# pbluc/avrecode-ms

Measured on AMD Instinct MI355X. Metric: H.264 bytes/s recompressed (CABAC re-encode of recorded bin streams, bit-exact vs CPU), higher is better.
Workload: dtype u32

## Files before the change

### avrecode-ms_amd/csrc/avr_k1p.h

```cpp
#pragma once
#include <stdint.h>

#include "avr_chunk.h"

#if defined(__HIPCC__)
#define AVR_HD __host__ __device__ inline
#else
#define AVR_HD inline
#endif

namespace avr {
namespace k1p {

#if defined(__HIP_DEVICE_COMPILE__)
#define AVR_PIN2(a, b) asm volatile("" : "+v"(a), "+v"(b))
#else
#define AVR_PIN2(a, b) ((void)0)
#endif

constexpr uint32_t kNone = 0xffffffffu;
constexpr uint32_t kMaxStretch = 16 * kChunk;
constexpr uint32_t kCodeBypass = 252;
constexpr uint32_t kCodePad = 252;

// ... 217 lines not shown
    if (chunk == 0) {
        o->first = 0;
        R[0] = R[1] = R[2] = R[3] = 510;
        i = 0;
    } else {
        uint32_t f = kNone;
        const uint32_t hi = limit < n ? limit : n;
        for_codes(res, lo, hi, [&](uint32_t idx, uint32_t c) { if (code_is_boundary(c)) { f = idx; return true; } return false; });
        if (f == kNone) {
            o->first = kNone; o->end = 0;
            for (int q = 0; q < 4; q++) { o->t_exit[q] = 0; o->r_exit[q] = 0; }
            return;
        }
        o->first = f;
        const uint32_t row = codes[res[f]].row;
        for (uint32_t q = 0; q < 4; q++) { uint32_t sh; R[q] = post_lps_range(row, q, &sh); }
        i = f + 1;
    }
    bool closed = false;
    auto merged = [&]() { return R[0] == R[1] && R[1] == R[2] && R[2] == R[3]; };
    auto code_by_code = [&](uint32_t stop) {
        if (i >= stop) return;
        uint32_t i_next = stop;
        for_codes(res, i, stop, [&](uint32_t idx, uint32_t c) {
            if (merged()) { i_next = idx; return true; }
            const bool closing = idx >= limit && code_is_boundary(c);
            if (closing)
                for (uint32_t q = 0; q < 4; q++) o->exit_q |= uint8_t(((R[q] >> 6) & 3) << (2 * q));
            const CodeEntry e = codes[c];
            for (uint32_t q = 0; q < 4; q++) T[q] += step_range(e, &R[q]);
            i_next = idx + 1;
            if (closing) { closed = true; return true; }
            return false;
        });
        i = i_next;
    };
    {
        const uint32_t interior_end = limit < n ? limit : n;
        const uint32_t a16 = (i + 15) & ~15u;
        code_by_code(a16 < interior_end ? a16 : interior_end);
        while (!merged() && i + 16 <= interior_end) {
            const U4 v = *reinterpret_cast<const U4 *>(res + i);
            const uint32_t w[4] = {v.x, v.y, v.z, v.w};
#if defined(__HIP_DEVICE_COMPILE__)
#pragma unroll 1
#endif
            for (uint32_t k = 0; k < 4; k++) {
                CodeEntry e[4];
                code_entries4(codes, w[k], e);
                for (uint32_t b = 0; b < 4; b++)
                    for (uint32_t q = 0; q < 4; q++) T[q] += step_range(e[b], &R[q]);
            }
            i += 16;
        }
        code_by_code(n);
    }
    uint32_t Rm = R[0], Tm = 0, end = i;
    if (!closed && i < n) {
        const uint32_t interior_end = limit < n ? limit : n;
        if (i < interior_end) {
            for_codes_all(res, i, interior_end, [&](uint32_t c) { Tm += step_range(codes[c], &Rm); },
                          [&](uint32_t d) {
                              CodeEntry e[4];
                              code_entries4(codes, d, e);
                              Tm += step_range(e[0], &Rm); Tm += step_range(e[1], &Rm);
                              Tm += step_range(e[2], &Rm); Tm += step_range(e[3], &Rm);
                          });
            i = interior_end;
        }
        end = n;
        for_codes(res, i, n, [&](uint32_t idx, uint32_t c) {
            const bool closing = idx >= limit && code_is_boundary(c);
            if (closing) o->exit_q = uint8_t(((Rm >> 6) & 3) * 0x55u);
            Tm += step_range(codes[c], &Rm);
            if (closing) { end = idx + 1; return true; }
            if (idx - lo > max_stretch) { o->too_long = 1; end = idx + 1; return true; }
            return false;
        });
        R[0] = R[1] = R[2] = R[3] = Rm;
    }
    o->end = end;
    for (uint32_t q = 0; q < 4; q++) { o->t_exit[q] = T[q] + Tm; o->r_exit[q] = uint16_t(R[q]); }
}


struct Entry {
    uint32_t t_start;
    uint32_t q;
};

struct SliceTotals {
    uint32_t t_total;
    uint32_t r_final;
    uint32_t bad;
    uint32_t pad;
};

AVR_HD void b2_chain(const Stretch *st, uint32_t n_chunks, Entry *en, SliceTotals *tot) {
    uint32_t T = 0, q = 0, r = 510, bad = 0;
    for (uint32_t c = 0; c < n_chunks; c++) {
        if (st[c].first == kNone) continue;
        en[c].t_start = T;
        en[c].q = q;
        T += st[c].t_exit[q];
        r = st[c].r_exit[q];
        bad |= st[c].too_long;
        q = (st[c].exit_q >> (2 * q)) & 3;
    }
    tot->t_total = T;
    tot->r_final = r;
    tot->bad = bad;
    tot->pad = 0;
}

AVR_HD uint32_t ref_digits(uint32_t t) { return t <= 21 ? 0 : (t - 21 + 15) / 16; }


template <class A, class = void> struct adder_is_staged { static constexpr bool value = false; };
template <class A> struct adder_is_staged<A, decltype(void(A::kStaged))> { static constexpr bool value = A::kStaged; };
template <class Src, class Adder>
AVR_HD void c_stretch_in(const Src &src, const Stretch &st, const Entry &en, uint32_t chunk,
                         const CodeEntryC *codes, Adder &S) {
    uint32_t R, from;
    if (chunk == 0) { R = 510; from = 0; }
    else { uint32_t sh; R = post_lps_range(codes[src.byte(st.first)].row, en.q, &sh); from = st.first + 1; }
    const uint32_t phase = en.t_start & 15, g0 = en.t_start >> 4;
    uint64_t L2 = 0;
    int sp = int(phase) - 7;
    uint32_t j = 0;
    constexpr bool staged = adder_is_staged<Adder>::value;
    if constexpr (staged) S.begin(g0);
    auto bin_e = [&](const CodeEntryC &e) {
        uint32_t v;
        const uint32_t sh = step_range_c(e, &R, &v);
        L2 = (L2 + v) << sh;
        sp += int(sh);
    };
    auto bin = [&](uint32_t c) { bin_e(codes[c]); };
    auto put = [&](uint32_t d) {
        if constexpr (staged) S.push(g0 + j, d);
        else if (j < 2) S.add(g0 + j, d);
        else S.store(g0 + j, d);
        j++;
    };
    auto digits = [&]() {
        while (sp >= 15) {
            const uint32_t d = uint32_t(L2 >> (sp + 1));
            L2 &= (uint64_t(2) << sp) - 1;
            put(d);
            sp -= 16;
        }
    };
    auto digits2 = [&]() {
        const int s1 = sp + 1;
        const uint32_t nd = uint32_t(s1 > 0 ? s1 : 0) >> 4, ks = 16 + (uint32_t(s1) & 15u);
        const uint64_t t = L2 >> ks;
        const uint32_t a = nd == 2 ? uint32_t(t >> 16) : uint32_t(t), b = uint32_t(t) & 0xffffu;
        L2 = uint32_t(L2) & (nd ? (1u << ks) - 1 : ~0u);
        sp -= int(16 * nd);
        if constexpr (staged) { S.push2(nd, a, b); j += nd; S.look(g0 + j); }
        else { if (nd) put(a); if (nd == 2) put(b); }
    };
    const uint32_t to = st.end;
    if (from < to) {
        auto four = [&](uint32_t d) {
            CodeEntryC e[4];
// ... 76 lines not shown
```

### avrecode-ms_amd/csrc/avr_k1p.hip

```cpp
#include <hip/hip_runtime.h>

#include <mutex>
#include <stdint.h>
#include <stdlib.h>
#include <type_traits>

#include "avr_coder.h"
#include "avr_internal.h"
#include "avr_k1p.h"
#include "avr_tables.h"

namespace avr {

static __device__ const CabacTables d_tables = make_cabac_tables();

using namespace k1p;

struct Plan {
    const uint16_t *recs;
    const uint64_t *rec_off;
    const uint32_t *n_bins;
    const uint64_t *res_off;
    const uint32_t *chunk_base, *chunk_slice;
    const uint32_t *blk_base, *blk_slice;
// ... 384 lines not shown
    uint64_t bits0 = 0, bits1 = 0;
    ChainAhead ahead(lbits, lend, nk, k, c0);
    ahead.walk(n_ch, [&](const ChainAhead::Chunk &c) {
        if (st[0] == st[1]) {
            *eo = uint8_t(st[0]);
            met_chunk = met_chunk < at ? met_chunk : at;
            if (at < 0xffffu) n_bins = kSegBits + 1u;
        }
        eo += row4;
        at++;
        const uint32_t cnt = c.cnt;
        const bool room = n_bins < kSegBits && cnt;
        if (__any(room) && room) {
            const uint32_t sh = c.pos & 31u;
            const uint64_t lo = uint64_t(__builtin_amdgcn_alignbit(c.w.y, c.w.x, sh)) | uint64_t(__builtin_amdgcn_alignbit(c.w.z, c.w.y, sh)) << 32;
            const uint64_t got = cnt < 64u ? lo & ((uint64_t(1) << cnt) - 1) : lo;
            if (n_bins < 64u) { bits0 |= got << n_bins; bits1 |= n_bins ? got >> (64u - n_bins) : 0u; }
            else bits1 |= got << (n_bins - 64u);
        }
        n_bins += cnt > 64u ? kSegBits + 1u : cnt;
        chain_step<2>(tn, c.bw, c.pos, cnt, c.w, st);
    });
    SegSummary o;
    o.bits[0] = bits0; o.bits[1] = bits1; o.n_bins = n_bins; o.exit_state = uint8_t(st[0]); o.met = st[0] == st[1] && met_chunk < 0xffffu;
    o.met_chunk = uint16_t(met_chunk < 0xffffu ? met_chunk : 0xffffu);
    summ[(size_t(L.s) * nk + k) * n_segs + L.seg] = o;
}

template <bool NOTE>
__device__ __forceinline__ uint32_t chain_chunks(const uint8_t *tn, const uint32_t *lbits, const uint16_t *lend, uint8_t *est, uint32_t nk, uint32_t row4,
                                                 uint32_t k, uint32_t c_first, uint32_t n_ch, uint32_t st0) {
    uint8_t *eo = est + size_t(c_first) * row4 + k;
    uint32_t st[1] = {st0};
    ChainAhead ahead(lbits, lend, nk, k, c_first);
    ahead.walk(n_ch, [&](const ChainAhead::Chunk &c) {
        if (NOTE) { *eo = uint8_t(st[0]); eo += row4; }
        chain_step<1>(tn, c.bw, c.pos, st[0] < 126u ? c.cnt : 0u, c.w, st);
    });
    return st[0];
}

__global__ __launch_bounds__(64 * kSegWaves) void k_k1p_chain_fix(Plan p, uint32_t n_slices, uint32_t n_segs, const int32_t *status,
                                                       const uint8_t *tng, const uint32_t *lbits, const uint16_t *lend, const uint8_t *init_states,
                                                       uint8_t *est, const SegSummary *summ, uint8_t *final_states, uint32_t force_walk_every) {
    __shared__ uint8_t tn[kTnBytes];
    for (uint32_t i = threadIdx.x; i < kTnBytes / 16; i += 64 * kSegWaves) reinterpret_cast<uint4 *>(tn)[i] = reinterpret_cast<const uint4 *>(tng)[i];
    __syncthreads();
    ChainLane L;
    if (!chain_lane(p, n_slices, n_segs, status, &L)) return;
    const uint32_t nk = p.n_states, row4 = ((nk + 3) >> 2) << 2, k = L.k;
    const SegSummary *mine = summ + (size_t(L.s) * nk + k) * n_segs;
    const uint32_t init = init_states[size_t(L.s) * p.ns_full + L.col] & 127u;
    const uint32_t c_slice = p.chunk_base[L.s], seg_len = (L.nc + n_segs - 1) / n_segs;
    const bool distrust = force_walk_every && (L.s * nk + k) % force_walk_every == 0;
    uint32_t from = L.seg, entry = init;
    if (init < 126u) {
        while (from > 0 && (distrust || !mine[from - 1].met)) from--;
        if (from > 0) entry = mine[from - 1].exit_state;
        for (uint32_t g = from; g < L.seg; g++) {
            const SegSummary sg = mine[g];
            if (sg.n_bins <= kSegBits && !distrust) {
                uint64_t b = sg.bits[0], b_hi = sg.bits[1];
                for (uint32_t left = sg.n_bins; left;) {
                    const uint32_t n = left < 8u ? left : 8u;
                    entry = tn[(128u << n) - 128u + (entry << n) + (uint32_t(b) & ((1u << n) - 1u))];
                    b = (b >> 8) | (b_hi << 56); b_hi >>= 8; left -= n;
                }
            } else {
                const uint32_t g_begin = g * seg_len < L.nc ? g * seg_len : L.nc, g_end = g_begin + seg_len < L.nc ? g_begin + seg_len : L.nc;
                entry = chain_chunks<false>(tn, lbits, lend, est, nk, row4, k, c_slice + g_begin, g_end - g_begin, entry);
            }
        }
    }
    const SegSummary me = mine[L.seg];
    const uint32_t n_ch = L.c_end - L.c_begin;
    const bool met = me.met && init < 126u && !distrust;
    const uint32_t stop = met && me.met_chunk < n_ch ? me.met_chunk : n_ch;
    const uint32_t exit_state = chain_chunks<true>(tn, lbits, lend, est, nk, row4, k, c_slice + L.c_begin, stop, entry);
    if (final_states && (L.c_end == L.nc) && (L.c_begin < L.nc || L.seg == 0))
        final_states[size_t(L.s) * p.ns_full + L.col] = uint8_t(stop < n_ch ? me.exit_state : exit_state);
}

__device__ __forceinline__ CodeEntry device_code_entry(uint32_t c);
__device__ __forceinline__ uint2 device_codes2(uint32_t c);

constexpr uint32_t kStBypass = 128, kStTerminate = 129, kStPad = 130, kStNone = 131, kReplayStates = 132;

typedef uint16_t u16x2 __attribute__((ext_vector_type(2)));
__device__ __forceinline__ uint32_t pk_sub(uint32_t a, uint32_t b) { return __builtin_bit_cast(uint32_t, __builtin_bit_cast(u16x2, a) - __builtin_bit_cast(u16x2, b)); }
__device__ __forceinline__ uint32_t pk_add(uint32_t a, uint32_t b) { return __builtin_bit_cast(uint32_t, __builtin_bit_cast(u16x2, a) + __builtin_bit_cast(u16x2, b)); }
__device__ __forceinline__ uint32_t pk_shl(uint32_t a, uint32_t b) { return __builtin_bit_cast(uint32_t, __builtin_bit_cast(u16x2, a) << __builtin_bit_cast(u16x2, b)); }
__device__ __forceinline__ uint32_t pk_shr8(uint32_t a) { return (a >> 8) & 0x00ff00ffu; }
__device__ __forceinline__ uint32_t step_pair(uint32_t &Rp, uint32_t row, uint32_t rown, uint32_t shrow, bool sym, uint32_t extra) {
    const uint32_t sel = ((Rp >> 6) & 0x00030003u) | 0x0c000c00u;
    const uint32_t rl = __builtin_amdgcn_perm(row, row, sel);
    const uint32_t rm = pk_sub(Rp, rl);
    const uint32_t shm = pk_shr8(rm) ^ 0x00010001u;
    const uint32_t rn = __builtin_amdgcn_perm(rown, rown, sel) | 0x01000100u;
    const uint32_t shl = __builtin_amdgcn_perm(shrow, shrow, sel);
    Rp = sym ? rn : pk_shl(rm, shm);
    return (sym ? shl : shm) + extra;
}

struct B1Walk {
    uint32_t i0, i1, limit, n, max_stretch;
    const uint2 *codes2;
    uint32_t mode, Rp0, Rp1, Tp0, Tp1, T[4], Rm, Tm, end;
    bool merged;
    Stretch o;

    __device__ __forceinline__ void init(uint32_t chunk, uint32_t i0_, uint32_t i1_, uint32_t n_, uint32_t max_stretch_, const uint2 *codes2_) {
        i0 = i0_; i1 = i1_; limit = i0_ + kChunk; n = n_; max_stretch = max_stretch_; codes2 = codes2_;
        mode = 0; Rp0 = Rp1 = 0x01fe01feu; Tp0 = Tp1 = 0; T[0] = T[1] = T[2] = T[3] = 0; Rm = 510; Tm = 0; end = 0;
        merged = false;
        o.first = kNone; o.end = 0; o.exit_q = 0; o.too_long = 0; o.pad[0] = o.pad[1] = 0;
        for (int q = 0; q < 4; q++) { o.t_exit[q] = 0; o.r_exit[q] = 0; }
        if (chunk == 0) { o.first = 0; mode = 2; merged = true; }
    }
    __device__ __forceinline__ void flush_t() {
        T[0] += Tp0 & 0xffffu; T[1] += Tp0 >> 16; T[2] += Tp1 & 0xffffu; T[3] += Tp1 >> 16;
        Tp0 = Tp1 = 0;
    }
    __device__ __forceinline__ bool met() const { return Rp0 == Rp1 && (Rp0 >> 16) == (Rp0 & 0xffffu); }
    __device__ __forceinline__ void one(uint32_t idx, const uint4 &e) {
        const CodeEntry ce{e.x, e.y >> 16};
        const bool boundary = ce.meta & 1u;
        if (mode == 0) {
            if (idx < i1 && boundary) {
                o.first = idx;
                const uint32_t rown = codes2[(e.y >> 8) & 0xffu].x;
                Rp0 = __builtin_amdgcn_perm(rown, rown, 0x0c010c00u) | 0x01000100u;
                Rp1 = __builtin_amdgcn_perm(rown, rown, 0x0c030c02u) | 0x01000100u;
                mode = 1;
            }
        } else if (mode == 1) {
            const bool closing = idx >= limit && boundary;
            if (closing)
                o.exit_q |= uint8_t(((Rp0 >> 6) & 3u) | ((Rp0 >> 22) & 3u) << 2 | ((Rp1 >> 6) & 3u) << 4 | ((Rp1 >> 22) & 3u) << 6);
            const uint2 e2 = codes2[(e.y >> 8) & 0xffu];
            const uint32_t extra = (ce.meta >> 8) * 0x00010001u;
            Tp0 = pk_add(Tp0, step_pair(Rp0, ce.row, e2.x, e2.y, boundary, extra));
            Tp1 = pk_add(Tp1, step_pair(Rp1, ce.row, e2.x, e2.y, boundary, extra));
            if (closing) { end = idx + 1; mode = 3; }
            else if (met()) { Rm = Rp0 & 0xffffu; mode = 2; merged = true; }
        } else if (mode == 2) {
            const bool closing = idx >= limit && boundary;
            if (closing) o.exit_q = uint8_t(((Rm >> 6) & 3) * 0x55u);
            Tm += step_merged(e);
            if (closing) { end = idx + 1; mode = 3; }
            else if (idx >= limit && idx - i0 > max_stretch) { o.too_long = 1; end = idx + 1; mode = 3; }
        }
    }
    __device__ __forceinline__ uint32_t step_merged(const uint4 &e) {
        uint32_t v;
        return step_range_c(CodeEntryC{e.x, e.z, 0u, e.w}, &Rm, &v);
    }
    __device__ __forceinline__ void group(uint32_t base, const uint4 e[8]) {
        if (mode == 2 && base + 8 <= i1) {
#pragma unroll
            for (uint32_t j = 0; j < 8; j++) Tm += step_merged(e[j]);
        } else if (mode == 1 && base + 8 <= i1) {
#pragma unroll
            for (uint32_t j = 0; j < 8; j++) {
                const uint2 e2 = codes2[(e[j].y >> 8) & 0xffu];
                const bool sym = (e[j].y >> 16) & 1u;
                const uint32_t extra = (e[j].y >> 24) * 0x00010001u;
                Tp0 = pk_add(Tp0, step_pair(Rp0, e[j].x, e2.x, e2.y, sym, extra));
                Tp1 = pk_add(Tp1, step_pair(Rp1, e[j].x, e2.x, e2.y, sym, extra));
            }
            flush_t();
            if (met()) { Rm = Rp0 & 0xffffu; mode = 2; merged = true; }
        } else if (mode != 3) {
            for (uint32_t j = 0; j < 8; j++) if (base + j < n) one(base + j, e[j]);
            flush_t();
        }
    }
    __device__ __forceinline__ void chunk_done() { if (mode == 0) mode = 3; }
    __device__ __forceinline__ void tail(uint32_t base, const uint4 e[8]) {
        for (uint32_t j = 0; j < 8; j++) if (base + j < n && mode != 3) one(base + j, e[j]);
        flush_t();
    }
    __device__ __forceinline__ const Stretch &finish() {
        if (o.first != kNone) {
            o.end = mode != 3 ? n : end;
            for (uint32_t q = 0; q < 4; q++) {
                const uint32_t rq = ((q & 2u) ? Rp1 : Rp0) >> (16 * (q & 1u)) & 0xffffu;
                o.t_exit[q] = T[q] + (merged ? Tm : 0u);
                o.r_exit[q] = uint16_t(merged ? Rm : rq);
            }
        }
        return o;
    }
};

template <bool TILE_CODES, bool R8>
__global__ __launch_bounds__(256) void k_k1p_replay(Plan p, uint32_t total_chunks, const uint32_t *est, uint8_t *res,
                                                    const int32_t *status, Stretch *stretch, uint32_t max_stretch) {
    extern __shared__ uint32_t replay_lds[];
    __shared__ uint4 info[2 * kReplayStates];
    __shared__ uint2 codes2[256];
    constexpr uint32_t kSelOff = R8 ? 128 : 2048;
    __shared__ uint32_t sel_off[kSelOff];
    const uint32_t lane = threadIdx.x & 63, nk = p.n_states;
    for (uint32_t c = threadIdx.x; c < 256; c += blockDim.x) codes2[c] = device_codes2(c);
    uint8_t *stb = reinterpret_cast<uint8_t *>(replay_lds) + (threadIdx.x >> 6) * (((nk + 8) >> 2) << 8) + lane * 4;
    for (uint32_t sel = threadIdx.x; sel < kSelOff; sel += blockDim.x) {
        uint32_t kk;
        if (R8) {
            kk = sel < nk ? sel : sel == AVR_SEL8_BYPASS ? nk + 1 : sel == AVR_SEL8_TERMINATE ? nk + 2 : nk + 4;
        } else {
            const uint32_t kLast = AVR_MAX_STATES - 1, over = (sel < kLast ? kLast : sel > kLast + 4 ? kLast + 4 : sel) - kLast;
            const uint32_t dense = sel < AVR_MAX_STATES ? uint32_t(p.table[sel]) : kNotUsed;
            kk = (dense < nk ? dense : nk) + over;
        }
        sel_off[sel] = ((kk & ~3u) << 6) + (kk & 3u);
    }
    for (uint32_t i = threadIdx.x; i < 2 * kReplayStates; i += blockDim.x) {
        const uint32_t st = i >> 1, bin = i & 1u;
        uint32_t next, code;
        if (st < 128) {
            const uint32_t nx = d_tables.packed[st][1];
            next = ((bin ^ st) & 1u) ? (nx >> 8) & 0xffu : nx & 0xffu;
            code = code_context(st, bin);
        } else {
            next = st;
            code = st == kStBypass ? kCodeBypass | bin : st == kStTerminate ? code_terminate(bin) : kCodePad;
        }
        const CodeEntry ce = device_code_entry(code);
        const CodeEntryC cc = code_entry_c(ce);
        info[i] = make_uint4(ce.row, next | code << 8 | ce.meta << 16, cc.side, cc.adj);
    }
    __syncthreads();
    const uint32_t gc = blockIdx.x * blockDim.x + threadIdx.x;
    if (gc >= total_chunks) return;
    const uint32_t s = p.chunk_slice[gc];
    Stretch o;
    o.first = kNone; o.end = 0; o.exit_q = 0; o.too_long = 0; o.pad[0] = o.pad[1] = 0;
    for (int q = 0; q < 4; q++) { o.t_exit[q] = 0; o.r_exit[q] = 0; }
    if (status[s] != AVR_SLICE_OK) { stretch[gc] = o; return; }
    const uint32_t c = gc - p.chunk_base[s];
    const uint32_t n = p.n_bins[s];
    const ChunkSpan span = chunk_span(c, n);
    const uint32_t i0 = span.i0, i1 = span.i1;
    {
        const uint32_t nkw = (nk + 3) >> 2;
        const uint32_t *e = est + size_t(gc) * nkw;
        for (uint32_t kw = 0; kw < nkw; kw++) *reinterpret_cast<uint32_t *>(stb + kw * 256) = e[kw];
        const uint32_t pseudo[5] = {kStNone, kStBypass, kStTerminate, kStPad, kStNone};
#pragma unroll
        for (uint32_t j = 0; j < 5; j++) stb[((nk + j) >> 2) * 256 + ((nk + j) & 3)] = uint8_t(pseudo[j]);
    }
    const uint16_t *r = p.recs + p.rec_off[s];
    uint8_t *ro = TILE_CODES ? res + TileCodes::group_at(gc, 0) : res + p.res_off[s];
    auto put16 = [&](uint32_t i, const U4 &v) {
        if (TILE_CODES) *reinterpret_cast<U4 *>(ro + size_t((i - i0) >> 4) * kTileRowBytes) = v;
        else *reinterpret_cast<U4 *>(ro + i) = v;
    };
    B1Walk b1;
    b1.init(c, i0, i1, n, max_stretch, codes2);
    auto eight = [&](const U4 &v, uint32_t &c0, uint32_t &c1, uint4 e[8]) {
        const uint32_t w[4] = {v.x, v.y, v.z, v.w};
        uint32_t off[8];
#pragma unroll
        for (uint32_t j = 0; j < 8; j++) off[j] = sel_off[((w[j >> 1] >> ((j & 1) * 16)) >> 1) & 0x7ffu];
#pragma unroll
        for (uint32_t j = 0; j < 8; j++) {
            const uint32_t bin = (w[j >> 1] >> ((j & 1) * 16)) & 1u;
            uint8_t *sp = stb + off[j];
            const uint32_t st = *sp;
            e[j] = info[(st << 1) | bin];
            *sp = uint8_t(e[j].y);
        }
        c0 = __builtin_amdgcn_perm(e[1].y, e[0].y, 0x0c0c0501u) | __builtin_amdgcn_perm(e[3].y, e[2].y, 0x05010c0cu);
        c1 = __builtin_amdgcn_perm(e[5].y, e[4].y, 0x0c0c0501u) | __builtin_amdgcn_perm(e[7].y, e[6].y, 0x05010c0cu);
    };
    if (R8) {
        const uint32_t pad_off = (((nk + 3) & ~3u) << 6) + ((nk + 3) & 3u);
        auto eight8 = [&](uint32_t lo, uint32_t hi, uint32_t base, uint32_t lim, auto masked, uint32_t &c0, uint32_t &c1, uint4 e[8]) {
            uint32_t off[8], bin[8];
#pragma unroll
            for (uint32_t j = 0; j < 8; j++) {
                const uint32_t b = ((j < 4 ? lo : hi) >> (8 * (j & 3))) & 0xffu;
                off[j] = sel_off[b >> 1];
                if (decltype(masked)::value) off[j] = base + j < lim ? off[j] : pad_off;
                bin[j] = b & 1u;
            }
#pragma unroll
            for (uint32_t j = 0; j < 8; j++) {
                uint8_t *sp = stb + off[j];
                const uint32_t st = *sp;
                e[j] = info[(st << 1) | bin[j]];
                *sp = uint8_t(e[j].y);
            }
            c0 = __builtin_amdgcn_perm(e[1].y, e[0].y, 0x0c0c0501u) | __builtin_amdgcn_perm(e[3].y, e[2].y, 0x05010c0cu);
            c1 = __builtin_amdgcn_perm(e[5].y, e[4].y, 0x0c0c0501u) | __builtin_amdgcn_perm(e[7].y, e[6].y, 0x05010c0cu);
        };
        auto sixteen8 = [&](uint32_t base, const U4 &v, auto masked) {
            U4 a;
            uint4 e[8];
            eight8(v.x, v.y, base, i1, masked, a.x, a.y, e); b1.group(base, e);
            eight8(v.z, v.w, base + 8, i1, masked, a.z, a.w, e); b1.group(base + 8, e);
            put16(base, a);
        };
        const uint8_t *r8 = p.recs8 + (p.rec_off[s] & ~uint64_t(15));
        if (i0 < n) {
            for_record_groups8(r8, i0, i1, sixteen8);
            b1.chunk_done();
            for (uint32_t i = i0 + kChunk; b1.mode != 3 && i < n; i += 8) {
                const uint2 v = *reinterpret_cast<const uint2 *>(r8 + i);
                uint32_t c0, c1;
                uint4 e[8];
                eight8(v.x, v.y, i, n, std::true_type{}, c0, c1, e);
                b1.tail(i, e);
            }
        }
        stretch[gc] = b1.finish();
        return;
    }
    uint32_t i = i0;
    if (i0 < n) {
        U4 v0{0, 0, 0, 0}, v1 = v0, v2 = v0, v3 = v0;
        const uint32_t last = i + 32 <= i1 ? i0 + ((i1 - i0) / 32u - 1u) * 32u : i0;
        if (i + 32 <= i1) {
            const U4 *q = reinterpret_cast<const U4 *>(r + i);
            v0 = q[0]; v1 = q[1]; v2 = q[2]; v3 = q[3];
        }
        for (; i + 32 <= i1; i += 32) {
            const U4 *qn = reinterpret_cast<const U4 *>(r + (i + 32 <= last ? i + 32 : last));
            const U4 n0 = qn[0], n1 = qn[1], n2 = qn[2], n3 = qn[3];
            U4 a, b;
            uint4 e[8];
            eight(v0, a.x, a.y, e); b1.group(i, e);
            eight(v1, a.z, a.w, e); b1.group(i + 8, e);
            eight(v2, b.x, b.y, e); b1.group(i + 16, e);
            eight(v3, b.z, b.w, e); b1.group(i + 24, e);
            put16(i, a);
            put16(i + 16, b);
            v0 = n0; v1 = n1; v2 = n2; v3 = n3;
        }
        for (; i < i1; i += 16) {
            const U4 *q = reinterpret_cast<const U4 *>(r + i);
            const U4 nop{AVR_NOP_CABAC2, AVR_NOP_CABAC2, AVR_NOP_CABAC2, AVR_NOP_CABAC2};
            const U4 t0 = q[0], t1 = i + 8 < i1 ? q[1] : nop;
            U4 a;
            uint4 e[8];
            eight(t0, a.x, a.y, e); b1.group(i, e);
            eight(t1, a.z, a.w, e); b1.group(i + 8, e);
            put16(i, a);
        }
        b1.chunk_done();
        for (i = i0 + kChunk; b1.mode != 3 && i < n; i += 8) {
            uint32_t c0, c1;
            uint4 e[8];
            eight(*reinterpret_cast<const U4 *>(r + i), c0, c1, e);
            b1.tail(i, e);
        }
    }
    stretch[gc] = b1.finish();
}


__device__ __forceinline__ CodeEntry device_code_entry(uint32_t c) {
    if (code_is_bypass(c)) return CodeEntry{0u, 0x100u | ((c & 1u) << 1)};
    return CodeEntry{d_tables.packed[2 * (c >> 2)][0], code_sym(c) * 3u};
}

__device__ __forceinline__ uint2 device_codes2(uint32_t c) {
    const uint32_t row = device_code_entry(c).row;
    uint32_t rown = 0, shrow = 0;
    for (uint32_t q = 0; q < 4; q++) {
        const uint32_t rl = (row >> (8 * q)) & 0xffu;
        if (rl) { uint32_t sh; const uint32_t rn = post_lps_range(row, q, &sh); rown |= (rn & 0xffu) << (8 * q); shrow |= sh << (8 * q); }
    }
    return make_uint2(rown, shrow);
}

__global__ __launch_bounds__(256) void k_k1p_b1(Plan p, uint32_t total_chunks, const uint8_t *res,
                                                const int32_t *status, Stretch *st, uint32_t max_stretch, uint8_t *tile) {
    __shared__ uint4 cinfo[256];
    __shared__ uint2 codes2[256];
    {
        const CodeEntry ce = device_code_entry(threadIdx.x);
        const CodeEntryC cc = code_entry_c(ce);
        cinfo[threadIdx.x] = make_uint4(ce.row, threadIdx.x << 8 | ce.meta << 16, cc.side, cc.adj);
        codes2[threadIdx.x] = device_codes2(threadIdx.x);
    }
    __syncthreads();
    const uint32_t gc = blockIdx.x * 256 + threadIdx.x;
    if (gc >= total_chunks) return;
    const uint32_t slice = p.chunk_slice[gc];
    if (status[slice] != AVR_SLICE_OK) { st[gc].first = kNone; st[gc].too_long = 0; return; }
    const uint32_t c = gc - p.chunk_base[slice], n = p.n_bins[slice];
    const ChunkSpan span = chunk_span(c, n);
    const uint32_t i0 = span.i0, i1 = span.i1;
    const uint8_t *r = res + p.res_off[slice];
    B1Walk b1;
    b1.init(c, i0, i1, n, max_stretch, codes2);
    auto eight = [&](uint32_t lo, uint32_t hi, uint4 e[8]) {
#pragma unroll
        for (uint32_t j = 0; j < 8; j++) e[j] = cinfo[((j < 4 ? lo : hi) >> (8 * (j & 3))) & 0xffu];
    };
    uint8_t *to = tile ? tile + TileCodes::group_at(gc, 0) : nullptr;
    auto sixteen = [&](uint32_t base, const U4 &v) {
        if (to) *reinterpret_cast<U4 *>(to + size_t((base - i0) >> 4) * kTileRowBytes) = v;
        uint4 e[8];
        eight(v.x, v.y, e); b1.group(base, e);
        eight(v.z, v.w, e); b1.group(base + 8, e);
    };
    uint32_t i = i0;
    if (i0 < n) {
        U4 v0{0, 0, 0, 0}, v1 = v0, v2 = v0, v3 = v0;
        if (i + 64 <= i1) { const U4 *q = reinterpret_cast<const U4 *>(r + i); v0 = q[0]; v1 = q[1]; v2 = q[2]; v3 = q[3]; }
        for (; i + 64 <= i1; i += 64) {
            const U4 *qn = reinterpret_cast<const U4 *>(r + (i + 128 <= i1 ? i + 64 : i));
            const U4 n0 = qn[0], n1 = qn[1], n2 = qn[2], n3 = qn[3];
            sixteen(i, v0); sixteen(i + 16, v1); sixteen(i + 32, v2); sixteen(i + 48, v3);
            v0 = n0; v1 = n1; v2 = n2; v3 = n3;
        }
        for (; i < i1; i += 16) sixteen(i, *reinterpret_cast<const U4 *>(r + i));
        b1.chunk_done();
        for (i = i0 + kChunk; b1.mode != 3 && i < n; i += 16) {
            const U4 v = *reinterpret_cast<const U4 *>(r + i);
            uint4 e[8];
            eight(v.x, v.y, e); b1.tail(i, e);
            if (b1.mode != 3) { eight(v.z, v.w, e); b1.tail(i + 8, e); }
        }
    }
    st[gc] = b1.finish();
}

constexpr uint32_t kB2Tile = 1024, kB2Seg = 16;

__global__ __launch_bounds__(256) void k_k1p_b2(Plan p, const int32_t *status, const Stretch *st, Entry *en,
                                                SliceTotals *tot, uint32_t *S) {
    __shared__ Stretch tile[kB2Tile];
    __shared__ Entry ent[kB2Tile];
    __shared__ uint8_t xq[kB2Tile], qin[kB2Tile];
    __shared__ uint8_t segmap[256], segin[kB2Tile / kB2Seg];
    __shared__ uint32_t wsum[4];
    __shared__ uint32_t carry[4];
    const uint32_t s = blockIdx.x, t = threadIdx.x, lane = t & 63, w = t >> 6;
    if (status[s] != AVR_SLICE_OK) {
        if (t == 0) { tot[s].t_total = 0; tot[s].r_final = 510; tot[s].bad = 0; tot[s].pad = 0; }
        return;
    }
    const uint32_t c0 = p.chunk_base[s], nc = p.chunk_base[s + 1] - c0;
    if (t == 0) { carry[0] = 0; carry[1] = 0; carry[2] = 510; carry[3] = 0; }
    for (uint32_t base = 0; base < nc; base += kB2Tile) {
        const uint32_t cnt = nc - base < kB2Tile ? nc - base : kB2Tile;
        const uint32_t *src = reinterpret_cast<const uint32_t *>(st + c0 + base);
        uint32_t *dst = reinterpret_cast<uint32_t *>(tile);
        for (uint32_t i = t; i < cnt * (sizeof(Stretch) / 4); i += 256) dst[i] = src[i];
        __syncthreads();
        for (uint32_t c = t; c < kB2Tile; c += 256) xq[c] = c < cnt && tile[c].first != kNone ? tile[c].exit_q : uint8_t(0xE4);
        __syncthreads();
        {
            const uint32_t seg = t >> 2, c_lo = seg * kB2Seg;
            uint32_t q = t & 3u;
            for (uint32_t c = c_lo; c < c_lo + kB2Seg; c++) q = (xq[c] >> (2 * q)) & 3;
            segmap[t] = uint8_t(q);
        }
        __syncthreads();
        if (t == 0) {
            uint32_t q = carry[1];
            for (uint32_t sg = 0; sg < kB2Tile / kB2Seg; sg++) { segin[sg] = uint8_t(q); q = segmap[4 * sg + q]; }
            carry[1] = q;
        }
        __syncthreads();
        if (t < kB2Tile / kB2Seg) {
            uint32_t q = segin[t];
            for (uint32_t c = t * kB2Seg; c < (t + 1) * kB2Seg; c++) { qin[c] = uint8_t(q); q = (xq[c] >> (2 * q)) & 3; }
        }
        __syncthreads();
        uint32_t tv[4], sum = 0, bad = 0, last = kNone;
#pragma unroll
        for (uint32_t j = 0; j < 4; j++) {
            const uint32_t c = 4 * t + j;
            const bool on = c < cnt && tile[c].first != kNone;
            tv[j] = on ? tile[c].t_exit[qin[c]] : 0;
            sum += tv[j];
            if (on) { bad |= tile[c].too_long; last = c; }
        }
        uint32_t incl = sum;
        for (uint32_t d = 1; d < 64; d <<= 1) { const uint32_t v = __shfl_up(incl, d); if (lane >= d) incl += v; }
        if (lane == 63) wsum[w] = incl;
        const uint64_t has = __ballot(last != kNone);
        __syncthreads();
        uint32_t run = carry[0] + incl - sum;
        for (uint32_t v = 0; v < w; v++) run += wsum[v];
#pragma unroll
        for (uint32_t j = 0; j < 4; j++) {
            const uint32_t c = 4 * t + j;
            if (c < cnt) { ent[c].t_start = run; ent[c].q = qin[c]; }
            run += tv[j];
        }
        if (bad) atomicOr(&carry[3], 1u);
        __syncthreads();
        if (t == 255) carry[0] = run;
        for (uint32_t v = 0; v < 4; v++) {
            if (w == v && has && lane == 63 - uint32_t(__builtin_clzll(has))) carry[2] = tile[last].r_exit[qin[last]];
            __syncthreads();
        }
        uint32_t *eo = reinterpret_cast<uint32_t *>(en + c0 + base);
        const uint32_t *ei = reinterpret_cast<const uint32_t *>(ent);
        for (uint32_t i = t; i < cnt * (sizeof(Entry) / 4); i += 256) eo[i] = ei[i];
        __syncthreads();
// ... 500 lines not shown
```

Baseline: 25.75 billion.

## Restructure B1 walk with branchless group stepping, vectorized open and tail paths

Moves the B1Walk state machine into a host/device header and rewrites its inner loops. Groups of eight bins now use branch-free select-based stepping. Boundary search in mode 0 uses a bitmask and ctz (open8), so the per-bin 'one' loop no longer runs while searching for a stretch start. Merged tails step eight bins predicated in one pass (tail8), and known-interior groups skip bounds checks through group_inside. The aim is to cut warp divergence and per-bin branching in the chunk-walk kernels, at the cost of doing redundant work on masked lanes and a more complex bit-exact state machine.

```diff
diff --git a/avrecode-ms_amd/csrc/avr_k1p.h b/avrecode-ms_amd/csrc/avr_k1p.h
--- a/avrecode-ms_amd/csrc/avr_k1p.h
+++ b/avrecode-ms_amd/csrc/avr_k1p.h
@@ -323,6 +323,226 @@
     o->end = end;
     for (uint32_t q = 0; q < 4; q++) { o->t_exit[q] = T[q] + Tm; o->r_exit[q] = uint16_t(R[q]); }
 }
+
+
+struct alignas(8) U2 { uint32_t x, y; };
+
+AVR_HD uint32_t perm_b32(uint32_t s0, uint32_t s1, uint32_t sel) {
+#if defined(__HIP_DEVICE_COMPILE__)
+    return __builtin_amdgcn_perm(s0, s1, sel);
+#else
+    const uint64_t both = uint64_t(s0) << 32 | s1;
+    uint32_t r = 0;
+    for (uint32_t i = 0; i < 4; i++) {
+        const uint32_t b = (sel >> (8 * i)) & 0xffu;
+        if (b < 8) r |= uint32_t((both >> (8 * b)) & 0xffu) << (8 * i);
+    }
+    return r;
+#endif
+}
+#if defined(__HIP_DEVICE_COMPILE__)
+typedef uint16_t u16x2 __attribute__((ext_vector_type(2)));
+AVR_HD uint32_t pk_sub(uint32_t a, uint32_t b) { return __builtin_bit_cast(uint32_t, __builtin_bit_cast(u16x2, a) - __builtin_bit_cast(u16x2, b)); }
+AVR_HD uint32_t pk_add(uint32_t a, uint32_t b) { return __builtin_bit_cast(uint32_t, __builtin_bit_cast(u16x2, a) + __builtin_bit_cast(u16x2, b)); }
+AVR_HD uint32_t pk_shl(uint32_t a, uint32_t b) { return __builtin_bit_cast(uint32_t, __builtin_bit_cast(u16x2, a) << __builtin_bit_cast(u16x2, b)); }
+AVR_HD uint32_t pk_shr(uint32_t a, uint32_t n) { return __builtin_bit_cast(uint32_t, __builtin_bit_cast(u16x2, a) >> __builtin_bit_cast(u16x2, n * 0x00010001u)); }
+#else
+AVR_HD uint32_t pk_halves(uint32_t lo, uint32_t hi) { return (lo & 0xffffu) | hi << 16; }
+AVR_HD uint32_t pk_sub(uint32_t a, uint32_t b) { return pk_halves((a & 0xffffu) - (b & 0xffffu), (a >> 16) - (b >> 16)); }
+AVR_HD uint32_t pk_add(uint32_t a, uint32_t b) { return pk_halves((a & 0xffffu) + (b & 0xffffu), (a >> 16) + (b >> 16)); }
+AVR_HD uint32_t pk_shl(uint32_t a, uint32_t b) { return pk_halves((a & 0xffffu) << (b & 15u), (a >> 16) << ((b >> 16) & 15u)); }
+AVR_HD uint32_t pk_shr(uint32_t a, uint32_t n) { return pk_halves((a & 0xffffu) >> n, (a >> 16) >> n); }
+#endif
+
+AVR_HD U4 b1_entry(const CodeEntry &ce, uint32_t next, uint32_t code) {
+    const CodeEntryC cc = code_entry_c(ce);
+    return U4{ce.row, next | code << 8 | ce.meta << 16, cc.side, cc.adj};
+}
+AVR_HD U2 codes2_entry(uint32_t row) {
+    U2 r{0, 0};
+    for (uint32_t q = 0; q < 4; q++) {
+        if (!((row >> (8 * q)) & 0xffu)) continue;
+        uint32_t sh;
+        const uint32_t rn = post_lps_range(row, q, &sh);
+        r.x |= (rn & 0xffu) << (8 * q);
+        r.y |= sh << (8 * q);
+    }
+    return r;
+}
+
+AVR_HD uint32_t step_pair(uint32_t &Rp, uint32_t row, uint32_t rown, uint32_t shrow, uint32_t side) {
+    const uint32_t sel = pk_shr(Rp, 6);
+    const uint32_t rl = perm_b32(row, 0u, sel);
+    const uint32_t rm = pk_sub(Rp, rl);
+    const uint32_t shm = pk_shr(rm, 8) ^ 0x00010001u;
+    const uint32_t rn = perm_b32(rown, 1u, sel);
+    const uint32_t shl = perm_b32(shrow, 0u, sel);
+    Rp = (rn & side) | (pk_shl(rm, shm) & ~side);
+    return (shl & side) | (shm & ~side);
+}
+
+struct B1Walk {
+    uint32_t i0, i1, limit, n, max_stretch;
+    const U2 *codes2;
+    uint32_t mode, Rp0, Rp1, Tp0, Tp1, T[4], end;
+    bool merged;
+    Stretch o;
+
+    AVR_HD void init(uint32_t chunk, uint32_t i0_, uint32_t i1_, uint32_t n_, uint32_t max_stretch_, const U2 *codes2_) {
+        i0 = i0_; i1 = i1_; limit = i0_ + kChunk; n = n_; max_stretch = max_stretch_; codes2 = codes2_;
+        mode = 0; Rp0 = Rp1 = 0x01fe01feu; Tp0 = Tp1 = 0; T[0] = T[1] = T[2] = T[3] = 0; end = 0;
+        merged = false;
+        o.first = kNone; o.end = 0; o.exit_q = 0; o.too_long = 0; o.pad[0] = o.pad[1] = 0;
+        for (int q = 0; q < 4; q++) { o.t_exit[q] = 0; o.r_exit[q] = 0; }
+        if (chunk == 0) { o.first = 0; Rp0 = 510; mode = 2; merged = true; }
+    }
+    AVR_HD void flush_t(uint32_t byp = 0) {
+        T[0] += (Tp0 & 0xffffu) + byp; T[1] += (Tp0 >> 16) + byp; T[2] += (Tp1 & 0xffffu) + byp; T[3] += (Tp1 >> 16) + byp;
+        Tp0 = Tp1 = 0;
+    }
+    AVR_HD bool met() const { return Rp0 == Rp1 && (Rp0 >> 16) == (Rp0 & 0xffffu); }
+    AVR_HD void join() { Rp0 &= 0xffffu; T[1] -= T[0]; T[2] -= T[0]; T[3] -= T[0]; mode = 2; merged = true; }
+    AVR_HD void open(uint32_t rown) {
+        Rp0 = perm_b32(rown, 1u, 0x00050004u);
+        Rp1 = perm_b32(rown, 1u, 0x00070006u);
+    }
+    AVR_HD uint32_t step_merged(const U4 &e) {
+        uint32_t v;
+        return step_range_c(CodeEntryC{e.x, e.z, 0u, e.w}, &Rp0, &v);
+    }
+    AVR_HD void one(uint32_t idx, const U4 &e) {
+        const bool boundary = (e.y >> 16) & 1u;
+        if (mode == 0) {
+            if (idx < i1 && boundary) { o.first = idx; open(codes2[(e.y >> 8) & 0xffu].x); mode = 1; }
+        } else if (mode == 1) {
+            const bool closing = idx >= limit && boundary;
+            if (closing)
+                o.exit_q |= uint8_t(((Rp0 >> 6) & 3u) | ((Rp0 >> 22) & 3u) << 2 | ((Rp1 >> 6) & 3u) << 4 | ((Rp1 >> 22) & 3u) << 6);
+            const U2 e2 = codes2[(e.y >> 8) & 0xffu];
+            const uint32_t extra = (e.y >> 24) * 0x00010001u;
+            Tp0 = pk_add(Tp0, step_pair(Rp0, e.x, e2.x, e2.y, e.z) + extra);
+            Tp1 = pk_add(Tp1, step_pair(Rp1, e.x, e2.x, e2.y, e.z) + extra);
+            if (closing) { end = idx + 1; mode = 3; }
+            else if (met()) { flush_t(); join(); }
+        } else if (mode == 2) {
+            const bool closing = idx >= limit && boundary;
+            if (closing) o.exit_q = uint8_t(((Rp0 >> 6) & 3) * 0x55u);
+            T[0] += step_merged(e);
+            if (closing) { end = idx + 1; mode = 3; }
+            else if (idx >= limit && idx - i0 > max_stretch) { o.too_long = 1; end = idx + 1; mode = 3; }
+        }
+    }
+    AVR_HD void merged8(const U4 e[8]) {
+#pragma unroll
+        for (uint32_t j = 0; j < 8; j++) T[0] += step_merged(e[j]);
+    }
+    AVR_HD void rows4(const U4 e[4], U2 r[4]) const {
+#pragma unroll
+        for (uint32_t j = 0; j < 4; j++) r[j] = codes2[(e[j].y >> 8) & 0xffu];
+        AVR_PIN2(r[0].x, r[0].y); AVR_PIN2(r[1].x, r[1].y); AVR_PIN2(r[2].x, r[2].y); AVR_PIN2(r[3].x, r[3].y);
+    }
+    AVR_HD void cand8(const U4 e[8]) {
+        uint32_t w = 8 * 23u;
+#pragma unroll
+        for (uint32_t h = 0; h < 8; h += 4) {
+            U2 r[4];
+            rows4(e + h, r);
+#pragma unroll
+            for (uint32_t j = 0; j < 4; j++) {
+                Tp0 = pk_add(Tp0, step_pair(Rp0, e[h + j].x, r[j].x, r[j].y, e[h + j].z));
+                Tp1 = pk_add(Tp1, step_pair(Rp1, e[h + j].x, r[j].x, r[j].y, e[h + j].z));
+                w += e[h + j].w;
+            }
+        }
+        flush_t(w);
+        if (met()) join();
+    }
+    AVR_HD void open8(uint32_t base, const U4 e[8]) {
+        uint32_t bm = 0;
+#pragma unroll
+        for (uint32_t j = 0; j < 8; j++) bm |= e[j].z & (1u << j);
+        const uint32_t at = mode == 0 ? uint32_t(__builtin_ctz(bm | 0x100u)) : kNone;
+        uint32_t w = 0;
+#pragma unroll
+        for (uint32_t h = 0; h < 8; h += 4) {
+            U2 r[4];
+            rows4(e + h, r);
+#pragma unroll
+            for (uint32_t j = 0; j < 4; j++) {
+                Tp0 = pk_add(Tp0, step_pair(Rp0, e[h + j].x, r[j].x, r[j].y, e[h + j].z));
+                Tp1 = pk_add(Tp1, step_pair(Rp1, e[h + j].x, r[j].x, r[j].y, e[h + j].z));
+                w += e[h + j].w + 23u;
+                const bool here = at == h + j;
+                Rp0 = here ? perm_b32(r[j].x, 1u, 0x00050004u) : Rp0;
+                Rp1 = here ? perm_b32(r[j].x, 1u, 0x00070006u) : Rp1;
+                Tp0 = here ? 0u : Tp0; Tp1 = here ? 0u : Tp1; w = here ? 0u : w;
+            }
+        }
+        if (at < 8) { o.first = base + at; mode = 1; }
+        if (mode == 1) {
+            flush_t(w);
+            if (met()) join();
+        } else {
+            Tp0 = Tp1 = 0;
+        }
+    }
+    AVR_HD void group_inside_as(uint32_t base, const U4 e[8], bool any_looking) {
+        if (mode == 2) merged8(e);
+        else if (any_looking) open8(base, e);
+        else cand8(e);
+    }
+    AVR_HD void group_inside(uint32_t base, const U4 e[8]) { group_inside_as(base, e, AVR_ANY(mode == 0)); }
+    AVR_HD void group(uint32_t base, const U4 e[8]) {
+        if (base + 8 <= i1) {
+            group_inside(base, e);
+        } else if (mode != 3) {
+            for (uint32_t j = 0; j < 8; j++) if (base + j < n) one(base + j, e[j]);
+            flush_t();
+        }
+    }
+    AVR_HD void chunk_done() { if (mode == 0) mode = 3; }
+    AVR_HD void tail8(uint32_t base, const U4 e[8]) {
+        uint32_t bm = 0;
+#pragma unroll
+        for (uint32_t j = 0; j < 8; j++) bm |= e[j].z & (1u << j);
+        const uint32_t closes = uint32_t(__builtin_ctz(bm | 0x100u));
+        const uint32_t d = base - i0, far = max_stretch >= d ? max_stretch - d + 1 : 0;
+        const uint32_t left = n - base - 1 < 7u ? n - base - 1 : 7u;
+        const uint32_t stop = closes < far ? closes : far, last = stop < left ? stop : left;
+        uint32_t before = Rp0;
+#pragma unroll
+        for (uint32_t j = 0; j < 8; j++) {
+            const bool on = j <= last;
+            uint32_t r = Rp0, v;
+            const uint32_t sh = step_range_c(CodeEntryC{e[j].x, e[j].z, 0u, e[j].w}, &r, &v);
+            before = on ? Rp0 : before;
+            Rp0 = on ? r : Rp0;
+            T[0] += on ? sh : 0u;
+        }
+        if (last == closes) { o.exit_q = uint8_t(((before >> 6) & 3) * 0x55u); end = base + last + 1; mode = 3; }
+        else if (last == far) { o.too_long = 1; end = base + last + 1; mode = 3; }
+    }
+    AVR_HD void tail(uint32_t base, const U4 e[8]) {
+        if (base >= n) return;
+        if (mode == 2) {
+            tail8(base, e);
+        } else {
+            for (uint32_t j = 0; j < 8; j++) if (base + j < n && mode != 3) one(base + j, e[j]);
+            flush_t();
+        }
+    }
+    AVR_HD const Stretch &finish() {
+        if (o.first != kNone) {
+            o.end = mode != 3 ? n : end;
+            for (uint32_t q = 0; q < 4; q++) {
+                const uint32_t rq = ((q & 2u) ? Rp1 : Rp0) >> (16 * (q & 1u)) & 0xffffu;
+                o.t_exit[q] = merged && q ? T[0] + T[q] : T[q];
+                o.r_exit[q] = uint16_t(merged ? Rp0 : rq);
+            }
+        }
+        return o;
+    }
+};
 
 
 struct Entry {
diff --git a/avrecode-ms_amd/csrc/avr_k1p.hip b/avrecode-ms_amd/csrc/avr_k1p.hip
--- a/avrecode-ms_amd/csrc/avr_k1p.hip
+++ b/avrecode-ms_amd/csrc/avr_k1p.hip
@@ -490,127 +490,19 @@
 }
 
 __device__ __forceinline__ CodeEntry device_code_entry(uint32_t c);
-__device__ __forceinline__ uint2 device_codes2(uint32_t c);
 
 constexpr uint32_t kStBypass = 128, kStTerminate = 129, kStPad = 130, kStNone = 131, kReplayStates = 132;
-
-typedef uint16_t u16x2 __attribute__((ext_vector_type(2)));
-__device__ __forceinline__ uint32_t pk_sub(uint32_t a, uint32_t b) { return __builtin_bit_cast(uint32_t, __builtin_bit_cast(u16x2, a) - __builtin_bit_cast(u16x2, b)); }
-__device__ __forceinline__ uint32_t pk_add(uint32_t a, uint32_t b) { return __builtin_bit_cast(uint32_t, __builtin_bit_cast(u16x2, a) + __builtin_bit_cast(u16x2, b)); }
-__device__ __forceinline__ uint32_t pk_shl(uint32_t a, uint32_t b) { return __builtin_bit_cast(uint32_t, __builtin_bit_cast(u16x2, a) << __builtin_bit_cast(u16x2, b)); }
-__device__ __forceinline__ uint32_t pk_shr8(uint32_t a) { return (a >> 8) & 0x00ff00ffu; }
-__device__ __forceinline__ uint32_t step_pair(uint32_t &Rp, uint32_t row, uint32_t rown, uint32_t shrow, bool sym, uint32_t extra) {
-    const uint32_t sel = ((Rp >> 6) & 0x00030003u) | 0x0c000c00u;
-    const uint32_t rl = __builtin_amdgcn_perm(row, row, sel);
-    const uint32_t rm = pk_sub(Rp, rl);
-    const uint32_t shm = pk_shr8(rm) ^ 0x00010001u;
-    const uint32_t rn = __builtin_amdgcn_perm(rown, rown, sel) | 0x01000100u;
-    const uint32_t shl = __builtin_amdgcn_perm(shrow, shrow, sel);
-    Rp = sym ? rn : pk_shl(rm, shm);
-    return (sym ? shl : shm) + extra;
-}
-
-struct B1Walk {
-    uint32_t i0, i1, limit, n, max_stretch;
-    const uint2 *codes2;
-    uint32_t mode, Rp0, Rp1, Tp0, Tp1, T[4], Rm, Tm, end;
-    bool merged;
-    Stretch o;
-
-    __device__ __forceinline__ void init(uint32_t chunk, uint32_t i0_, uint32_t i1_, uint32_t n_, uint32_t max_stretch_, const uint2 *codes2_) {
-        i0 = i0_; i1 = i1_; limit = i0_ + kChunk; n = n_; max_stretch = max_stretch_; codes2 = codes2_;
-        mode = 0; Rp0 = Rp1 = 0x01fe01feu; Tp0 = Tp1 = 0; T[0] = T[1] = T[2] = T[3] = 0; Rm = 510; Tm = 0; end = 0;
-        merged = false;
-        o.first = kNone; o.end = 0; o.exit_q = 0; o.too_long = 0; o.pad[0] = o.pad[1] = 0;
-        for (int q = 0; q < 4; q++) { o.t_exit[q] = 0; o.r_exit[q] = 0; }
-        if (chunk == 0) { o.first = 0; mode = 2; merged = true; }
-    }
-    __device__ __forceinline__ void flush_t() {
-        T[0] += Tp0 & 0xffffu; T[1] += Tp0 >> 16; T[2] += Tp1 & 0xffffu; T[3] += Tp1 >> 16;
-        Tp0 = Tp1 = 0;
-    }
-    __device__ __forceinline__ bool met() const { return Rp0 == Rp1 && (Rp0 >> 16) == (Rp0 & 0xffffu); }
-    __device__ __forceinline__ void one(uint32_t idx, const uint4 &e) {
-        const CodeEntry ce{e.x, e.y >> 16};
-        const bool boundary = ce.meta & 1u;
-        if (mode == 0) {
-            if (idx < i1 && boundary) {
-                o.first = idx;
-                const uint32_t rown = codes2[(e.y >> 8) & 0xffu].x;
-                Rp0 = __builtin_amdgcn_perm(rown, rown, 0x0c010c00u) | 0x01000100u;
-                Rp1 = __builtin_amdgcn_perm(rown, rown, 0x0c030c02u) | 0x01000100u;
-                mode = 1;
-            }
-        } else if (mode == 1) {
-            const bool closing = idx >= limit && boundary;
-            if (closing)
-                o.exit_q |= uint8_t(((Rp0 >> 6) & 3u) | ((Rp0 >> 22) & 3u) << 2 | ((Rp1 >> 6) & 3u) << 4 | ((Rp1 >> 22) & 3u) << 6);
-            const uint2 e2 = codes2[(e.y >> 8) & 0xffu];
-            const uint32_t extra = (ce.meta >> 8) * 0x00010001u;
-            Tp0 = pk_add(Tp0, step_pair(Rp0, ce.row, e2.x, e2.y, boundary, extra));
-            Tp1 = pk_add(Tp1, step_pair(Rp1, ce.row, e2.x, e2.y, boundary, extra));
-            if (closing) { end = idx + 1; mode = 3; }
-            else if (met()) { Rm = Rp0 & 0xffffu; mode = 2; merged = true; }
-        } else if (mode == 2) {
-            const bool closing = idx >= limit && boundary;
-            if (closing) o.exit_q = uint8_t(((Rm >> 6) & 3) * 0x55u);
-            Tm += step_merged(e);
-            if (closing) { end = idx + 1; mode = 3; }
-            else if (idx >= limit && idx - i0 > max_stretch) { o.too_long = 1; end = idx + 1; mode = 3; }
-        }
-    }
-    __device__ __forceinline__ uint32_t step_merged(const uint4 &e) {
-        uint32_t v;
-        return step_range_c(CodeEntryC{e.x, e.z, 0u, e.w}, &Rm, &v);
-    }
-    __device__ __forceinline__ void group(uint32_t base, const uint4 e[8]) {
-        if (mode == 2 && base + 8 <= i1) {
-#pragma unroll
-            for (uint32_t j = 0; j < 8; j++) Tm += step_merged(e[j]);
-        } else if (mode == 1 && base + 8 <= i1) {
-#pragma unroll
-            for (uint32_t j = 0; j < 8; j++) {
-                const uint2 e2 = codes2[(e[j].y >> 8) & 0xffu];
-                const bool sym = (e[j].y >> 16) & 1u;
-                const uint32_t extra = (e[j].y >> 24) * 0x00010001u;
-                Tp0 = pk_add(Tp0, step_pair(Rp0, e[j].x, e2.x, e2.y, sym, extra));
-                Tp1 = pk_add(Tp1, step_pair(Rp1, e[j].x, e2.x, e2.y, sym, extra));
-            }
-            flush_t();
-            if (met()) { Rm = Rp0 & 0xffffu; mode = 2; merged = true; }
-        } else if (mode != 3) {
-            for (uint32_t j = 0; j < 8; j++) if (base + j < n) one(base + j, e[j]);
-            flush_t();
-        }
-    }
-    __device__ __forceinline__ void chunk_done() { if (mode == 0) mode = 3; }
-    __device__ __forceinline__ void tail(uint32_t base, const uint4 e[8]) {
-        for (uint32_t j = 0; j < 8; j++) if (base + j < n && mode != 3) one(base + j, e[j]);
-        flush_t();
-    }
-    __device__ __forceinline__ const Stretch &finish() {
-        if (o.first != kNone) {
-            o.end = mode != 3 ? n : end;
-            for (uint32_t q = 0; q < 4; q++) {
-                const uint32_t rq = ((q & 2u) ? Rp1 : Rp0) >> (16 * (q & 1u)) & 0xffffu;
-                o.t_exit[q] = T[q] + (merged ? Tm : 0u);
-                o.r_exit[q] = uint16_t(merged ? Rm : rq);
-            }
-        }
-        return o;
-    }
-};
 
 template <bool TILE_CODES, bool R8>
 __global__ __launch_bounds__(256) void k_k1p_replay(Plan p, uint32_t total_chunks, const uint32_t *est, uint8_t *res,
                                                     const int32_t *status, Stretch *stretch, uint32_t max_stretch) {
     extern __shared__ uint32_t replay_lds[];
-    __shared__ uint4 info[2 * kReplayStates];
-    __shared__ uint2 codes2[256];
+    __shared__ U4 info[2 * kReplayStates];
+    __shared__ U2 codes2[256];
     constexpr uint32_t kSelOff = R8 ? 128 : 2048;
     __shared__ uint32_t sel_off[kSelOff];
     const uint32_t lane = threadIdx.x & 63, nk = p.n_states;
-    for (uint32_t c = threadIdx.x; c < 256; c += blockDim.x) codes2[c] = device_codes2(c);
+    for (uint32_t c = threadIdx.x; c < 256; c += blockDim.x) codes2[c] = codes2_entry(device_code_entry(c).row);
     uint8_t *stb = reinterpret_cast<uint8_t *>(replay_lds) + (threadIdx.x >> 6) * (((nk + 8) >> 2) << 8) + lane * 4;
     for (uint32_t sel = threadIdx.x; sel < kSelOff; sel += blockDim.x) {
         uint32_t kk;
@@ -634,9 +526,7 @@
             next = st;
             code = st == kStBypass ? kCodeBypass | bin : st == kStTerminate ? code_terminate(bin) : kCodePad;
         }
-        const CodeEntry ce = device_code_entry(code);
-        const CodeEntryC cc = code_entry_c(ce);
-        info[i] = make_uint4(ce.row, next | code << 8 | ce.meta << 16, cc.side, cc.adj);
+        info[i] = b1_entry(device_code_entry(code), next, code);
     }
     __syncthreads();
     const uint32_t gc = blockIdx.x * blockDim.x + threadIdx.x;
@@ -666,7 +556,7 @@
     };
     B1Walk b1;
     b1.init(c, i0, i1, n, max_stretch, codes2);
-    auto eight = [&](const U4 &v, uint32_t &c0, uint32_t &c1, uint4 e[8]) {
+    auto eight = [&](const U4 &v, uint32_t &c0, uint32_t &c1, U4 e[8]) {
         const uint32_t w[4] = {v.x, v.y, v.z, v.w};
         uint32_t off[8];
 #pragma unroll
@@ -684,7 +574,7 @@
     };
     if (R8) {
         const uint32_t pad_off = (((nk + 3) & ~3u) << 6) + ((nk + 3) & 3u);
-        auto eight8 = [&](uint32_t lo, uint32_t hi, uint32_t base, uint32_t lim, auto masked, uint32_t &c0, uint32_t &c1, uint4 e[8]) {
+        auto eight8 = [&](uint32_t lo, uint32_t hi, uint32_t base, uint32_t lim, auto masked, uint32_t &c0, uint32_t &c1, U4 e[8]) {
             uint32_t off[8], bin[8];
 #pragma unroll
             for (uint32_t j = 0; j < 8; j++) {
@@ -705,9 +595,10 @@
         };
         auto sixteen8 = [&](uint32_t base, const U4 &v, auto masked) {
             U4 a;
-            uint4 e[8];
-            eight8(v.x, v.y, base, i1, masked, a.x, a.y, e); b1.group(base, e);
-            eight8(v.z, v.w, base + 8, i1, masked, a.z, a.w, e); b1.group(base + 8, e);
+            U4 e[8];
+            auto group = [&](uint32_t at) { if (decltype(masked)::value) b1.group(at, e); else b1.group_inside(at, e); };
+            eight8(v.x, v.y, base, i1, masked, a.x, a.y, e); group(base);
+            eight8(v.z, v.w, base + 8, i1, masked, a.z, a.w, e); group(base + 8);
             put16(base, a);
         };
         const uint8_t *r8 = p.recs8 + (p.rec_off[s] & ~uint64_t(15));
@@ -717,7 +608,7 @@
             for (uint32_t i = i0 + kChunk; b1.mode != 3 && i < n; i += 8) {
                 const uint2 v = *reinterpret_cast<const uint2 *>(r8 + i);
                 uint32_t c0, c1;
-                uint4 e[8];
+                U4 e[8];
                 eight8(v.x, v.y, i, n, std::true_type{}, c0, c1, e);
                 b1.tail(i, e);
             }
@@ -737,11 +628,11 @@
             const U4 *qn = reinterpret_cast<const U4 *>(r + (i + 32 <= last ? i + 32 : last));
             const U4 n0 = qn[0], n1 = qn[1], n2 = qn[2], n3 = qn[3];
             U4 a, b;
-            uint4 e[8];
-            eight(v0, a.x, a.y, e); b1.group(i, e);
-            eight(v1, a.z, a.w, e); b1.group(i + 8, e);
-            eight(v2, b.x, b.y, e); b1.group(i + 16, e);
-            eight(v3, b.z, b.w, e); b1.group(i + 24, e);
+            U4 e[8];
+            eight(v0, a.x, a.y, e); b1.group_inside(i, e);
+            eight(v1, a.z, a.w, e); b1.group_inside(i + 8, e);
+            eight(v2, b.x, b.y, e); b1.group_inside(i + 16, e);
+            eight(v3, b.z, b.w, e); b1.group_inside(i + 24, e);
             put16(i, a);
             put16(i + 16, b);
             v0 = n0; v1 = n1; v2 = n2; v3 = n3;
@@ -751,7 +642,7 @@
             const U4 nop{AVR_NOP_CABAC2, AVR_NOP_CABAC2, AVR_NOP_CABAC2, AVR_NOP_CABAC2};
             const U4 t0 = q[0], t1 = i + 8 < i1 ? q[1] : nop;
             U4 a;
-            uint4 e[8];
+            U4 e[8];
             eight(t0, a.x, a.y, e); b1.group(i, e);
             eight(t1, a.z, a.w, e); b1.group(i + 8, e);
             put16(i, a);
@@ -759,7 +650,7 @@
         b1.chunk_done();
         for (i = i0 + kChunk; b1.mode != 3 && i < n; i += 8) {
             uint32_t c0, c1;
-            uint4 e[8];
+            U4 e[8];
             eight(*reinterpret_cast<const U4 *>(r + i), c0, c1, e);
             b1.tail(i, e);
         }
@@ -773,25 +664,14 @@
     return CodeEntry{d_tables.packed[2 * (c >> 2)][0], code_sym(c) * 3u};
 }
 
-__device__ __forceinline__ uint2 device_codes2(uint32_t c) {
-    const uint32_t row = device_code_entry(c).row;
-    uint32_t rown = 0, shrow = 0;
-    for (uint32_t q = 0; q < 4; q++) {
-        const uint32_t rl = (row >> (8 * q)) & 0xffu;
-        if (rl) { uint32_t sh; const uint32_t rn = post_lps_range(row, q, &sh); rown |= (rn & 0xffu) << (8 * q); shrow |= sh << (8 * q); }
-    }
-    return make_uint2(rown, shrow);
-}
-
 __global__ __launch_bounds__(256) void k_k1p_b1(Plan p, uint32_t total_chunks, const uint8_t *res,
                                                 const int32_t *status, Stretch *st, uint32_t max_stretch, uint8_t *tile) {
-    __shared__ uint4 cinfo[256];
-    __shared__ uint2 codes2[256];
+    __shared__ U4 cinfo[256];
+    __shared__ U2 codes2[256];
     {
         const CodeEntry ce = device_code_entry(threadIdx.x);
-        const CodeEntryC cc = code_entry_c(ce);
-        cinfo[threadIdx.x] = make_uint4(ce.row, threadIdx.x << 8 | ce.meta << 16, cc.side, cc.adj);
-        codes2[threadIdx.x] = device_codes2(threadIdx.x);
+        cinfo[threadIdx.x] = b1_entry(ce, 0u, threadIdx.x);
+        codes2[threadIdx.x] = codes2_entry(ce.row);
     }
     __syncthreads();
     const uint32_t gc = blockIdx.x * 256 + threadIdx.x;
@@ -804,16 +684,17 @@
     const uint8_t *r = res + p.res_off[slice];
     B1Walk b1;
     b1.init(c, i0, i1, n, max_stretch, codes2);
-    auto eight = [&](uint32_t lo, uint32_t hi, uint4 e[8]) {
+    auto eight = [&](uint32_t lo, uint32_t hi, U4 e[8]) {
 #pragma unroll
         for (uint32_t j = 0; j < 8; j++) e[j] = cinfo[((j < 4 ? lo : hi) >> (8 * (j & 3))) & 0xffu];
     };
     uint8_t *to = tile ? tile + TileCodes::group_at(gc, 0) : nullptr;
-    auto sixteen = [&](uint32_t base, const U4 &v) {
+    auto sixteen = [&](uint32_t base, const U4 &v, auto inside) {
         if (to) *reinterpret_cast<U4 *>(to + size_t((base - i0) >> 4) * kTileRowBytes) = v;
-        uint4 e[8];
-        eight(v.x, v.y, e); b1.group(base, e);
-        eight(v.z, v.w, e); b1.group(base + 8, e);
+        U4 e[8];
+        auto group = [&](uint32_t at) { if (decltype(inside)::value) b1.group_inside(at, e); else b1.group(at, e); };
+        eight(v.x, v.y, e); group(base);
+        eight(v.z, v.w, e); group(base + 8);
     };
     uint32_t i = i0;
     if (i0 < n) {
@@ -822,14 +703,14 @@
         for (; i + 64 <= i1; i += 64) {
             const U4 *qn = reinterpret_cast<const U4 *>(r + (i + 128 <= i1 ? i + 64 : i));
             const U4 n0 = qn[0], n1 = qn[1], n2 = qn[2], n3 = qn[3];
-            sixteen(i, v0); sixteen(i + 16, v1); sixteen(i + 32, v2); sixteen(i + 48, v3);
+            sixteen(i, v0, std::true_type{}); sixteen(i + 16, v1, std::true_type{}); sixteen(i + 32, v2, std::true_type{}); sixteen(i + 48, v3, std::true_type{});
             v0 = n0; v1 = n1; v2 = n2; v3 = n3;
         }
-        for (; i < i1; i += 16) sixteen(i, *reinterpret_cast<const U4 *>(r + i));
+        for (; i < i1; i += 16) sixteen(i, *reinterpret_cast<const U4 *>(r + i), std::false_type{});
         b1.chunk_done();
         for (i = i0 + kChunk; b1.mode != 3 && i < n; i += 16) {
             const U4 v = *reinterpret_cast<const U4 *>(r + i);
-            uint4 e[8];
+            U4 e[8];
             eight(v.x, v.y, e); b1.tail(i, e);
             if (b1.mode != 3) { eight(v.z, v.w, e); b1.tail(i + 8, e); }
         }
```

After: 26.96 billion, median of 6. 4.7% higher.
